# amansanghvi/Thesis

Measured on AMD Instinct MI355X. Metric: particle-updates/sec (particles x scans/s) @1081 beams, higher is better.
Workload: dtype int8 map cells (lattice log-odds), f64 poses/weights; 1 GPU; BASELINE configs[2]: room16 synthetic, 4096 particles/GPU, 1081 beams, 0.05 m grid, K=30 samples, both matcher stages, resample every step; particles_per_gpu=4096, beams=1081, parallelism=particles sharded x1

## Files before the change

### include/rbpf_hip.h

```cpp
#ifndef RBPF_HIP_H
#define RBPF_HIP_H

#include <stdint.h>

#ifdef __cplusplus
extern "C" {
#endif

#define RBPF_OK 0
#define RBPF_EINVAL (-1)
#define RBPF_ENOMEM (-2)
#define RBPF_EDEVICE (-3)
#define RBPF_ESTATE (-4)
#define RBPF_ERANGE (-5)

#define RBPF_IMU_UNICYCLE 0
#define RBPF_IMU_ABSOLUTE 1
#define RBPF_IMU_VELOCITY 2

typedef struct rbpf_handle rbpf_handle;

typedef struct rbpf_config {
    int32_t n_particles;
    int32_t n_samples;
// ... 110 lines not shown
int32_t rbpf_pack_raw_width(rbpf_handle* h);
int32_t rbpf_pack_meta_width(rbpf_handle* h);
int  rbpf_gather_pack_meta(rbpf_handle* h, const int32_t* local_idx, int32_t n, void* d_raw);
int  rbpf_meta_from_raw(rbpf_handle* h, const int32_t* raw, int32_t n, int32_t* meta_out, int64_t* bytes_out);
int  rbpf_pack_particles_raw(rbpf_handle* h, const int32_t* local_idx, int32_t n, const int32_t* raw, void* d_buf,
                             int64_t cap_bytes, int64_t* bytes_out);

int  rbpf_get_poses(rbpf_handle* h, double* out_p3);
int  rbpf_get_covs(rbpf_handle* h, double* out_p9);
int  rbpf_get_weights(rbpf_handle* h, double* out_p);
int  rbpf_set_state(rbpf_handle* h, const double* poses_p3, const double* covs_p9,
                    const double* weights_p);
int  rbpf_get_rng_state(rbpf_handle* h, uint64_t* scan_updates, uint64_t* resample_draws);
int  rbpf_set_rng_state(rbpf_handle* h, uint64_t scan_updates, uint64_t resample_draws);
int  rbpf_get_tile_count(rbpf_handle* h, int32_t particle, int32_t* out_n);
int  rbpf_get_tile(rbpf_handle* h, int32_t particle, int32_t k, double* centre2, int8_t* cells);
int  rbpf_set_tile(rbpf_handle* h, int32_t particle, double cx, double cy, const int8_t* cells);
int  rbpf_get_dim(rbpf_handle* h, int32_t* out_dim);
int  rbpf_get_odds_at(rbpf_handle* h, int32_t particle, const double* xy, int32_t n,
                      double* out_vals, uint8_t* out_none);

#define RBPF_RENDER_DEVICE_OUT 1u
int  rbpf_map_extent(rbpf_handle* h, int32_t particle, int32_t* box4);
int  rbpf_render_map(rbpf_handle* h, int32_t particle, const int32_t* box4, const double* weights,
                     uint32_t flags, int8_t* cells, float* prob, float* occ_frac);

#define RBPF_LOAD_DEVICE_IN 1u
int  rbpf_load_map(rbpf_handle* h, int32_t particle, const int32_t* box4, const int8_t* cells, uint32_t flags);
#define RBPF_PLACE_DEVICE_IN  1u
#define RBPF_PLACE_DEVICE_OUT 2u
// ... 102 lines not shown
```

### thesis_amd/_lib.py

```python
from __future__ import annotations

import ctypes as C
import os

HERE = os.path.dirname(os.path.abspath(__file__))
LIB_PATH = os.path.join(HERE, "librbpf_hip.so")

RBPF_OK = 0
RBPF_EINVAL, RBPF_ENOMEM, RBPF_EDEVICE, RBPF_ESTATE, RBPF_ERANGE = -1, -2, -3, -4, -5
RBPF_RENDER_DEVICE_OUT = 1
RBPF_LOAD_DEVICE_IN = 1
RBPF_CAST_DEVICE_OUT = 1
RBPF_LOCATE_DEVICE_OUT = 1
RBPF_ALIGN_DEVICE_OUT = 1
RBPF_GAIN_DEVICE_OUT = 1
RBPF_TRAVEL_DEVICE_OUT, RBPF_TRAVEL_THROUGH_UNKNOWN = 1, 2
RBPF_FRONTIER_DEVICE_OUT = 1
RBPF_SCORE_DEVICE_IN, RBPF_SCORE_DEVICE_OUT, RBPF_SCORE_FIELDS = 1, 2, 13
RBPF_W_UNIFORM, RBPF_W_RESAMPLE, RBPF_W_GIVEN = 0, 1, 2
RBPF_EST_F64, RBPF_EST_I32 = 16, 4
RBPF_TRACK_IMU, RBPF_TRACK_SCAN, RBPF_TRACK_CHUNK, RBPF_TRACK_DEVICE_OUT = 1, 2, 64, 1
RBPF_BUILD_DEVICE_OUT, RBPF_BUILD_ACCUMULATE = 1, 2
RBPF_REFINE_DEVICE_OUT = 1
RBPF_PAIRS_DEVICE_OUT = 1
# ... 76 lines not shown
    "rbpf_apply_resample_local": (C.c_int, [_H, _I, _I]),
    "rbpf_set_global_ids": (C.c_int, [_H, _I]),
    "rbpf_pack_meta_width": (C.c_int32, [_H]),
    "rbpf_unpack_particles": (C.c_int, [_H, _I, C.c_int32, C.c_void_p, _I]),
    "rbpf_pack_raw_width": (C.c_int32, [_H]),
    "rbpf_gather_pack_meta": (C.c_int, [_H, _I, C.c_int32, C.c_void_p]),
    "rbpf_meta_from_raw": (C.c_int, [_H, _I, C.c_int32, _I, C.POINTER(C.c_int64)]),
    "rbpf_pack_particles_raw": (C.c_int, [_H, _I, C.c_int32, _I, C.c_void_p, C.c_int64, C.POINTER(C.c_int64)]),
    "rbpf_get_poses": (C.c_int, [_H, _D]),
    "rbpf_get_covs": (C.c_int, [_H, _D]),
    "rbpf_get_weights": (C.c_int, [_H, _D]),
    "rbpf_set_state": (C.c_int, [_H, _D, _D, _D]),
    "rbpf_get_rng_state": (C.c_int, [_H, C.POINTER(C.c_uint64), C.POINTER(C.c_uint64)]),
    "rbpf_set_rng_state": (C.c_int, [_H, C.c_uint64, C.c_uint64]),
    "rbpf_get_tile_count": (C.c_int, [_H, C.c_int32, _I]),
    "rbpf_get_tile": (C.c_int, [_H, C.c_int32, C.c_int32, _D, _B]),
    "rbpf_set_tile": (C.c_int, [_H, C.c_int32, C.c_double, C.c_double, _B]),
    "rbpf_get_dim": (C.c_int, [_H, _I]),
    "rbpf_get_odds_at": (C.c_int, [_H, C.c_int32, _D, C.c_int32, _D, _U]),
    "rbpf_map_extent": (C.c_int, [_H, C.c_int32, _I]),
    "rbpf_render_map": (C.c_int, [_H, C.c_int32, _I, _D, C.c_uint32, C.c_void_p, C.c_void_p, C.c_void_p]),
    "rbpf_load_map": (C.c_int, [_H, C.c_int32, _I, C.c_void_p, C.c_uint32]),
    "rbpf_place_map": (C.c_int, [_H, C.c_int32, _I, C.c_void_p, C.c_int32, C.c_int32, C.c_double, _D, C.c_int32, C.c_int32, C.c_uint32,
                       C.c_void_p, C.c_void_p]),
    "rbpf_set_map_updates": (C.c_int, [_H, C.c_int32]),
    "rbpf_get_map_updates": (C.c_int, [_H, _I]),
    "rbpf_get_map_update_workgroups": (C.c_int, [_H, _I]),
    "rbpf_cast_scans": (C.c_int, [_H, C.c_int32, _D, C.c_int32, _D, C.c_int32, C.c_double, C.c_uint32, C.c_void_p, C.c_void_p]),
    "rbpf_locate_scan": (C.c_int, [_H, C.c_int32, _I, _D, _D, C.c_int32, C.c_int32, C.c_uint32, C.c_void_p, C.c_void_p]),
    "rbpf_align_points": (C.c_int, [_H, C.c_int32, _I, _D, C.c_int32, _D, C.c_int32, C.c_int32, C.c_int32, C.c_int32, C.c_uint32,
# ... 86 lines not shown
```

### thesis_amd/csrc/kernels_resample.hip

```cpp
#include <limits.h>

#include "rbpf_internal.h"

namespace rbpf {

static const int PLAN_THREADS = 1024;

__device__ __forceinline__ dd dd_two_prod(double a, double b) {
    double p = a * b;
    double e = __fma_rn(a, b, -p);
    return {p, e};
}
__device__ __forceinline__ dd dd_mul_d(dd a, double b) {
    dd p = dd_two_prod(a.hi, b);
    double lo = p.lo + a.lo * b;
    double hi = p.hi + lo;
    return {hi, lo - (hi - p.hi)};
}
__device__ __forceinline__ dd dd_sub(dd a, dd b) { return dd_add(a, dd{-b.hi, -b.lo}); }
__device__ __forceinline__ dd dd_div_d(dd a, double b) {
    double q1 = a.hi / b;
    dd r = dd_sub(a, dd_two_prod(q1, b));
    double q2 = (r.hi + r.lo) / b;
    double hi = q1 + q2;
// ... 447 lines not shown
    if (tid == 0) { v.tile_bbox[4 * td + 0] = j.x0; v.tile_bbox[4 * td + 1] = j.x1; v.tile_bbox[4 * td + 2] = j.ya; v.tile_bbox[4 * td + 3] = j.yb - 1; }
}

__global__ __launch_bounds__(PLAN_THREADS) void resample_plan_kernel(ResampleArgs a) { resample_plan_stage(a); }
__global__ void resample_expand_kernel(int P, const int32_t* __restrict__ T, int32_t* __restrict__ idx) {
    const int j = blockIdx.x * blockDim.x + threadIdx.x;
    if (j < P) resample_expand_one(P, T, idx, j);
}
__global__ __launch_bounds__(PLAN_THREADS) void resample_pair_kernel(PairArgs a) { resample_pair_stage(a); }
__global__ __launch_bounds__(PLAN_THREADS) void sources_to_T_kernel(int P, const int32_t* __restrict__ idx, int32_t* __restrict__ T,
                                                                     int32_t* __restrict__ did) { sources_to_T_stage(P, idx, T, did); }

enum { RS_PLAN = 1, RS_SRC2T = 2, RS_EXPAND = 4, RS_PAIR = 8, RS_GATHER = 16 };
static const int RS_FUSE_MAX = 4096;
static const int RS_GATHER_FUSE_MAX = 1024;
struct FusedArgs { int stages; ResampleArgs ra; int32_t* idx; PairArgs pa; GatherArgs ga; };
__global__ __launch_bounds__(PLAN_THREADS) void resample_fused_kernel(FusedArgs f) {
    extern __shared__ __align__(16) int32_t s_dyn[];
    int32_t* const s_T = s_dyn; int32_t* const s_idx = s_dyn + RS_FUSE_MAX;
    const int tid = threadIdx.x, P = f.ra.P;
#ifdef RBPF_STAMPS
    long long st[6]; st[0] = clock64();
#define RSTAMP(k) st[k] = clock64()
#else
#define RSTAMP(k) do { } while (0)
#endif
    if (f.stages & RS_PLAN) { resample_plan_stage(f.ra); __syncthreads(); }
    RSTAMP(1);
    if (f.stages & RS_SRC2T) { sources_to_T_stage(P, f.idx, f.ra.T, f.ra.did); __syncthreads(); }
    for (int j = tid; j < P; j += PLAN_THREADS) s_T[j] = f.ra.T[j];
    __syncthreads();
    if (f.stages & RS_EXPAND) { for (int j = tid; j < P; j += PLAN_THREADS) { resample_expand_one(P, s_T, s_idx, j); f.idx[j] = s_idx[j]; } }
    else for (int j = tid; j < P; j += PLAN_THREADS) s_idx[j] = f.idx[j];
    __syncthreads();
    RSTAMP(2);
    if (f.stages & RS_PAIR) { PairArgs pa = f.pa; pa.T = s_T; pa.idx = s_idx; resample_pair_stage(pa); __syncthreads(); }
    RSTAMP(3);
    if (f.stages & RS_GATHER) { GatherArgs ga = f.ga; ga.T = s_T; ga.idx = s_idx; for (int j = tid; j < ga.P; j += PLAN_THREADS) resample_gather_one(ga, j); }
    RSTAMP(4);
#ifdef RBPF_STAMPS
    if (tid == 0) printf("resample_fused: plan %lld expand %lld pair %lld gather %lld cycles\n", st[1] - st[0], st[2] - st[1], st[3] - st[2], st[4] - st[3]);
#endif
}

static void launch_resample_fused(const FusedArgs& f, hipStream_t s) {
    const size_t lds = 2 * RS_FUSE_MAX * sizeof(int32_t);
    static size_t lds_set[MAX_DEVICES] = {};
    ensure_dynamic_lds(reinterpret_cast<const void*>(resample_fused_kernel), lds, lds_set);
    hipLaunchKernelGGL(resample_fused_kernel, dim3(1), dim3(PLAN_THREADS), lds, s, f);
}

void launch_export_weights(const DevView& v, double* d_out, int n_global, const uint8_t* d_bad, hipStream_t s) {
    (void)hipMemsetAsync(d_out, 0, (size_t)(n_global + (d_bad ? 1 : 0)) * 8, s);
    hipLaunchKernelGGL(export_weights_kernel, dim3((v.P + 255) / 256), dim3(256), 0, s, v.P, v.weight, v.global_id, d_out, n_global, d_bad);
// ... 3 lines not shown
    hipLaunchKernelGGL(gather_meta_kernel, dim3((tot + 255) / 256), dim3(256), 0, s, v, d_local, n, d_out);
}
void launch_pack(const DevView& v, const void* d_jobs, int n_jobs, void* d_buf, hipStream_t s) {
    if (n_jobs) hipLaunchKernelGGL(pack_kernel, dim3(n_jobs), dim3(BLOCK), 0, s, v, static_cast<const PackJob*>(d_jobs), static_cast<unsigned char*>(d_buf));
}
void launch_unpack(const DevView& v, const ResampleBuffers& b, const void* d_jobs, int n_jobs, const void* d_buf, hipStream_t s) {
    if (n_jobs) hipLaunchKernelGGL(unpack_kernel, dim3(n_jobs), dim3(BLOCK), 0, s, v, static_cast<const UnpackJob*>(d_jobs),
                                   static_cast<const unsigned char*>(d_buf), b.pending_free, b.n_pending);
    hipLaunchKernelGGL(resample_release_kernel, dim3(1), dim3(256), 0, s, v, b.pending_free, b.n_pending);
}

void launch_resample_indices(int P, const double* d_w, double u, double spread, int32_t* d_T, int32_t* d_idx,
                             int32_t* d_did, int32_t* d_err, hipStream_t s) {
    ResampleArgs ra{P, d_w, u, spread, d_T, d_did, d_err};
    if (P <= RS_FUSE_MAX) {
        FusedArgs f{RS_PLAN | RS_EXPAND, ra, d_idx, PairArgs{}, GatherArgs{}};
        launch_resample_fused(f, s);
        return;
    }
    hipLaunchKernelGGL(resample_plan_kernel, dim3(1), dim3(PLAN_THREADS), 0, s, ra);
    hipLaunchKernelGGL(resample_expand_kernel, dim3((P + 255) / 256), dim3(256), 0, s, P, d_T, d_idx);
}

void launch_resample_local(const DevView& v, const ResampleBuffers& b, const double* d_w, double u, double spread, hipStream_t s) {
    const PairArgs pa{v.P, b.T, b.idx, b.did, v.slot, b.slot2, b.dead_list, b.jobs, b.n_jobs, v.err};
    const GatherArgs ga{v.P, b.idx, b.did, v.px, v.py, v.pth, v.cov, v.weight, b.px2, b.py2, b.pth2, b.cov2, b.w2, b.T, v.dup_of};
    const bool fuse_gather = v.P <= RS_GATHER_FUSE_MAX;
    if (v.P > RS_FUSE_MAX) {
        if (d_w) launch_resample_indices(v.P, d_w, u, spread, b.T, b.idx, b.did, v.err, s);
        else hipLaunchKernelGGL(sources_to_T_kernel, dim3(1), dim3(PLAN_THREADS), 0, s, v.P, b.idx, b.T, b.did);
        hipLaunchKernelGGL(resample_pair_kernel, dim3(1), dim3(PLAN_THREADS), 0, s, pa);
    } else {
        FusedArgs f{(d_w ? RS_PLAN | RS_EXPAND : RS_SRC2T) | RS_PAIR | (fuse_gather ? RS_GATHER : 0),
                    ResampleArgs{v.P, d_w, u, spread, b.T, b.did, v.err}, b.idx, pa, ga};
        launch_resample_fused(f, s);
    }
    CopyArgs ca{v, b.jobs, b.n_jobs, b.pending_free, b.n_pending, fuse_gather ? 0 : 1, ga};
    hipLaunchKernelGGL(resample_copy_kernel, dim3(512), dim3(COPY_BLOCK), 0, s, ca);
    hipLaunchKernelGGL(resample_release_kernel, dim3(1), dim3(256), 0, s, v, b.pending_free, b.n_pending);
}

}
```

### thesis_amd/csrc/rbpf_api.hip

```cpp
#include <math.h>
#include <stdio.h>
#include <stdlib.h>
#include <string.h>

#include <algorithm>
#include <limits>

#include "rbpf_host.h"

using namespace rbpf;

static thread_local std::string g_create_err;

#define HIP_TRY(h, call)                                                                           \
    do {                                                                                           \
        hipError_t e_ = (call);                                                                    \
        if (e_ != hipSuccess) {                                                                    \
            (h)->err = std::string(#call) + ": " + hipGetErrorString(e_);                          \
            return RBPF_EDEVICE;                                                                   \
        }                                                                                          \
    } while (0)

struct DevGuard {
    int prev = -1; bool switched = false;
    explicit DevGuard(int dev) {
        if (hipGetDevice(&prev) != hipSuccess) { (void)hipGetLastError(); prev = -1; }
        if (prev != dev) { if (hipSetDevice(dev) == hipSuccess) switched = prev >= 0; else (void)hipGetLastError(); }
    }
    ~DevGuard() { if (switched) (void)hipSetDevice(prev); }
    DevGuard(const DevGuard&) = delete; DevGuard& operator=(const DevGuard&) = delete;
};
#define ON_DEVICE(h) DevGuard dev_guard_((h)->cfg.device)

static int fail(rbpf_handle* h, int code, const std::string& msg) {
    if (h) h->err = msg; else g_create_err = msg;
    return code;
}

template <typename T>
static int dev_alloc(rbpf_handle* h, T** out, size_t n) {
    h->allocs.emplace_back();
    hipError_t e = h->allocs.back().reserve(n * sizeof(T));
    if (e != hipSuccess) { h->err = std::string("hipMalloc: ") + hipGetErrorString(e); return RBPF_ENOMEM; }
    *out = h->allocs.back().as<T>();
    return RBPF_OK;
}
#define ALLOC(h, ptr, n) do { int rc_ = dev_alloc(h, &(ptr), (n)); if (rc_) return rc_; } while (0)
// ... 125 lines not shown
            double rel = pos - (double)lat * v.tile_len;
            int cidx = trunc_to_int(rel / v.cs + (double)dim / 2.0);
            if (cidx < 0 || cidx >= dim) { delete h; return fail(nullptr, RBPF_EINVAL, "cell index formula leaves the tile for this cell_size (the reference would raise IndexError)"); }
            if (g_first == INT32_MAX) g_first = g;
            uint32_t ent = ((uint32_t)(lat + v.R) << 16) | (uint32_t)cidx;
            if (!lut.empty() && ent < lut.back()) { delete h; return fail(nullptr, RBPF_EINVAL, "cell index formula is not monotone for this cell_size"); }
            lut.push_back(ent);
        }
        v.g_min = g_first; v.n_lut = (int)lut.size();
    }

    int rc = RBPF_OK;
    auto build = [&]() -> int {
        HIP_TRY(h, hipStreamCreateWithFlags(&h->stream, hipStreamNonBlocking));
        h->own_stream = true;
        for (int k = 0; k < rbpf_handle::N_KERN; ++k)
            for (int e = 0; e < 2; ++e) {
                h->ring[k][e].resize(rbpf_handle::RING);
                for (auto& ev : h->ring[k][e]) HIP_TRY(h, h->events.create(&ev, hipEventDisableSystemFence));
                h->begin_used[k].assign(rbpf_handle::RING, nullptr);
            }
        const size_t P = v.P, LL = (size_t)v.L * v.L, cells = (size_t)dim * dim;
        uint32_t* d_lut; ALLOC(h, d_lut, h->h_lut.size()); v.lut = d_lut;
        HIP_TRY(h, hipMemcpy(d_lut, h->h_lut.data(), h->h_lut.size() * 4, hipMemcpyHostToDevice));
        {
            const int KW = (dim + WIN - 1) / WIN;
            std::vector<int32_t> gw((size_t)v.L * (KW + 1));
            for (int a = 0; a < v.L; ++a)
                for (int k = 0; k <= KW; ++k) {
                    uint32_t key = k < KW ? (((uint32_t)a << 16) | (uint32_t)(k * WIN)) : ((uint32_t)(a + 1) << 16);
// ... 22 lines not shown
            v.wsel_x = reinterpret_cast<const float*>(d + 3 * MBP * 8 + 4 * MBP * 4 + MBP); v.wsel_y = v.wsel_x + MBW;
            v.wsel_idx = reinterpret_cast<const uint16_t*>(v.wsel_y + MBW);
            HIP_TRY(h, h->rings[R_SCAN].create(h->scan_bytes));
            HIP_TRY(h, h->rings[R_LAST].create(MB * 16));
            HIP_TRY(h, h->rings[R_IDX].create((size_t)P * 8));
        }
        ALLOC(h, v.upd_pose, 3 * P);
        ALLOC(h, v.prop_prep, 24 * P);
        ALLOC(h, v.prop_samp, 256 * P);
        ALLOC(h, v.stats, ST_COUNT); ALLOC(h, v.err, 1);
        ALLOC(h, v.mu_fallback, P); HIP_TRY(h, hipMemset(v.mu_fallback, 0, P * 4));
        ALLOC(h, v.ev_queue, 2); HIP_TRY(h, hipMemset(v.ev_queue, 0, 8));
        ALLOC(h, h->d_did_early, 1);
        HIP_TRY(h, hipMemset(h->d_did_early, 0, 4));
        HIP_TRY(h, h->events.create(&h->ev_weights, hipEventDisableTiming | hipEventDisableSystemFence));
        {
            v.mu_mode = env_is("RBPF_MAP_KERNEL", "window") ? MU_WINDOW : env_is("RBPF_MAP_KERNEL", "ray") ? MU_RAY : env_is("RBPF_MAP_KERNEL", "ev") ? MU_EV : MU_DEFAULT;
            v.ev_resident = env_is("RBPF_EV_RESIDENT", "0") ? 0 : 1;
            const char* eg = getenv("RBPF_EV_GRID");
            v.ev_grid = eg ? std::max(0, atoi(eg)) : 0;
            v.match_stage_slow = env_is("RBPF_MATCH_STAGE", "slow") ? 1 : 0;
            const char* ws = getenv("RBPF_WSAFE");
            v.wsafe_override = ws ? (float)atof(ws) : -1.0f;
            v.weight_entry_f64 = env_is("RBPF_WEIGHT_ENTRY", "f64") ? 1 : 0;
            v.ndt_refine = h->cfg.ndt_refine;
            h->dedup_enabled = !env_is("RBPF_MATCH_DEDUP", "0");
        }
        ALLOC(h, v.dup_of, P); v.dups_valid = 0;
        ALLOC(h, h->d_last_xy, 2 * (size_t)c.max_beams); ALLOC(h, h->d_tmp_sel, 2 * (size_t)c.max_beams);
        if (raycast_lds_bytes(c.max_beams, v.reach) > LDS_LIMIT) return fail(h, RBPF_EINVAL, "max_beams too large for the LDS window layout");
        match_geometry(c, c.cell_size, h->mN, h->mds, h->mmcs, h->md0, h->mncr);
        h->mlds = match_lds_bytes(h->mN, c.max_beams, match_max_coarse(h->mncr, 0.7, h->mmcs), match_per_rot(0.7, h->mmcs));
        if (h->mlds > LDS_LIMIT) return fail(h, RBPF_EINVAL, "matcher region does not fit in LDS for this cell_size");
        if (c.ndt_refine && ndt_cells(h->mmcs) >= 2) {
            if (ndt_lds_bytes(h->mN, c.max_beams) > LDS_LIMIT) return fail(h, RBPF_EINVAL, "NDT stage: matcher region does not fit in LDS");
            ALLOC(h, v.ndt_occ, P * (size_t)h->mN * (h->mN / 32)); ALLOC(h, v.ndt_aux, 5 * P);
        }
        ALLOC(h, h->d_match, 13 * P); ALLOC(h, h->d_bad, P); ALLOC(h, h->d_guess_full, P * (size_t)c.n_samples * 3);
        {
            ResampleBuffers& r = h->rs;
            ALLOC(h, r.T, P); ALLOC(h, r.idx, P); ALLOC(h, r.did, 1); ALLOC(h, r.slot2, P); ALLOC(h, r.dead_list, P);
            ALLOC(h, r.jobs, 2 * P); ALLOC(h, r.n_jobs, 2); ALLOC(h, r.pending_free, (size_t)v.pool_tiles); ALLOC(h, r.n_pending, 1);
            ALLOC(h, r.px2, P); ALLOC(h, r.py2, P); ALLOC(h, r.pth2, P); ALLOC(h, r.cov2, 9 * P); ALLOC(h, r.w2, P);
            HIP_TRY(h, hipMemset(r.n_pending, 0, 4)); HIP_TRY(h, hipMemset(r.n_jobs, 0, 8)); HIP_TRY(h, hipMemset(r.did, 0, 4));
        }
        HIP_TRY(h, hipMemset(v.pool, 0, (size_t)v.pool_tiles * cells));
        HIP_TRY(h, hipMemset(v.px, 0, P * 8)); HIP_TRY(h, hipMemset(v.py, 0, P * 8)); HIP_TRY(h, hipMemset(v.pth, 0, P * 8));
        HIP_TRY(h, hipMemset(v.cov, 0, 9 * P * 8));
        HIP_TRY(h, hipMemset(v.stats, 0, ST_COUNT * 8)); HIP_TRY(h, hipMemset(v.err, 0, 4));
        std::vector<double> w(P, 1.0);
        HIP_TRY(h, hipMemcpy(v.weight, w.data(), P * 8, hipMemcpyHostToDevice));
        std::vector<int32_t> ids(P), tab(P * LL, -1), fs(v.pool_tiles), bb((size_t)v.pool_tiles * 4);
        for (size_t p = 0; p < P; ++p) { ids[p] = (int32_t)p; tab[p * LL + (size_t)v.R * v.L + v.R] = (int32_t)p; }
        for (int t = 0; t < v.pool_tiles; ++t) { bb[4 * t] = INT32_MAX; bb[4 * t + 1] = -1; bb[4 * t + 2] = INT32_MAX; bb[4 * t + 3] = -1; }
        int32_t top = v.pool_tiles - (int32_t)P;
        for (int i = 0; i < top; ++i) fs[i] = v.pool_tiles - 1 - i;
        HIP_TRY(h, hipMemcpy(v.slot, ids.data(), P * 4, hipMemcpyHostToDevice));
        HIP_TRY(h, hipMemcpy(v.global_id, ids.data(), P * 4, hipMemcpyHostToDevice));
        HIP_TRY(h, hipMemcpy(v.tile_tab, tab.data(), P * LL * 4, hipMemcpyHostToDevice));
        HIP_TRY(h, hipMemcpy(v.free_stack, fs.data(), (size_t)v.pool_tiles * 4, hipMemcpyHostToDevice));
        HIP_TRY(h, hipMemcpy(v.free_top, &top, 4, hipMemcpyHostToDevice));
        HIP_TRY(h, hipMemcpy(v.tile_bbox, bb.data(), bb.size() * 4, hipMemcpyHostToDevice));
        return RBPF_OK;
    };
    rc = build();
    if (rc != RBPF_OK) { g_create_err = h->err; rbpf_destroy(h); return rc; }
    *out = h;
    return RBPF_OK;
}

int rbpf_destroy(rbpf_handle* h) {
    if (!h) return RBPF_OK;
    ON_DEVICE(h);
    if (hipStreamSynchronize(h->stream) != hipSuccess) (void)hipGetLastError();
    h->each_staging([](Staging& s) { if (s.wait() != hipSuccess) (void)hipGetLastError(); });
    if (h->ev_weights_valid && hipEventSynchronize(h->ev_weights) != hipSuccess) (void)hipGetLastError();
    for (Block& b : h->allocs) b.release();
    for (Block& b : h->buf) b.release();
    for (Block& b : h->track_mem) b.release();
    h->each_staging([](Staging& s) { s.release(); });
    h->each_staging([](Staging& s) { s.destroy_event(); });
    h->events.destroy();
    if (h->own_stream && h->stream) (void)hipStreamDestroy(h->stream);
    (void)hipGetLastError();
    delete h;
    return RBPF_OK;
}

const char* rbpf_last_error(const rbpf_handle* h) { return h ? h->err.c_str() : g_create_err.c_str(); }

int rbpf_set_stream(rbpf_handle* h, void* s) {
    if (!h) return RBPF_EINVAL;
    ON_DEVICE(h);
    HIP_TRY(h, hipStreamSynchronize(h->stream));
    if (h->own_stream && h->stream) (void)hipStreamDestroy(h->stream);
    h->own_stream = false;
    h->stream = static_cast<hipStream_t>(s);
    h->last_end = nullptr;
    return RBPF_OK;
}

int rbpf_release_stream(rbpf_handle* h) {
    if (!h) return RBPF_EINVAL;
    ON_DEVICE(h);
    if (h->own_stream) return RBPF_OK;
    HIP_TRY(h, hipStreamSynchronize(h->stream));
    if (h->early_n > 0) HIP_TRY(h, h->stage[S_EARLY].wait());
    h->stream = nullptr;
    HIP_TRY(h, hipStreamCreateWithFlags(&h->stream, hipStreamNonBlocking));
    h->own_stream = true;
    h->last_end = nullptr;
    return RBPF_OK;
}

int rbpf_abi_struct_bytes(int32_t* config_bytes, int32_t* counters_bytes) {
    if (config_bytes) *config_bytes = (int32_t)sizeof(rbpf_config);
    if (counters_bytes) *counters_bytes = (int32_t)sizeof(rbpf_counters);
    return RBPF_OK;
}

int rbpf_synchronize(rbpf_handle* h) {
    if (!h) return RBPF_EINVAL;
// ... 247 lines not shown
    }
    const double* d_g = nullptr;
    if (guesses) {
        HIP_TRY(h, hipMemcpyAsync(h->d_guess_full, guesses, P * (size_t)v.K * 3 * 8, hipMemcpyHostToDevice, h->stream));
        d_g = h->d_guess_full;
    }
    if (!match_override && !guesses) h->prof_begin_chained(1); else h->prof_begin(1);
    const int32_t* match_of = (!match_override && v.dups_valid) ? v.dup_of : nullptr;
    if (h->prop_capture && !h->d_prop_w) ALLOC(h, h->d_prop_w, P * (size_t)v.K);
    launch_propose_weight(v, h->d_match, match_of, d_g, h->d_bad, h->cfg.seed, (uint32_t)h->scan_updates, h->prop_capture ? h->d_prop_w : nullptr, h->stream);
    h->prop_valid = true; h->prop_captured = h->prop_capture;
    v.dups_valid = 0;
    h->prof_end(1);
    HIP_TRY(h, hipGetLastError());
    h->ev_weights_valid = false;
    if (h->record_ev_weights) { HIP_TRY(h, hipEventRecord(h->ev_weights, h->stream)); h->ev_weights_valid = true; }
    h->scan_begun = true; h->begin_seen = true;
    return RBPF_OK;
}

int rbpf_scan_update_end(rbpf_handle* h) {
    if (!h) return RBPF_EINVAL;
    ON_DEVICE(h);
    if (!h->scan_begun) return fail(h, RBPF_ESTATE, "rbpf_scan_update_begin has not been called");
    h->scan_begun = false;
    if (!h->map_updates) {
        launch_bad_weight(h->v, h->d_bad, h->stream);
        HIP_TRY(h, hipGetLastError());
        h->scan_updates++;
    } else {
        const int rc = run_map_update(h, h->d_bad);
        if (rc) return rc;
    }
    if (h->track_on && (h->track_flags & RBPF_TRACK_SCAN)) return track_record(h, true);
    return RBPF_OK;
}

int rbpf_set_proposal_capture(rbpf_handle* h, int32_t on) {
    if (!h) return RBPF_EINVAL;
    h->prop_capture = on != 0;
// ... 148 lines not shown

static double internal_uniform(rbpf_handle* h) {
    uint64_t z = h->cfg.seed + 0x9E3779B97F4A7C15ull * (++h->resample_draws);
    z = (z ^ (z >> 30)) * 0xBF58476D1CE4E5B9ull;
    z = (z ^ (z >> 27)) * 0x94D049BB133111EBull;
    z ^= z >> 31;
    return (double)(z >> 11) * (1.0 / 9007199254740992.0);
}

static void swap_state_buffers(rbpf_handle* h) {
    DevView& v = h->v; ResampleBuffers& r = h->rs;
    std::swap(v.px, r.px2); std::swap(v.py, r.py2); std::swap(v.pth, r.pth2);
    std::swap(v.cov, r.cov2); std::swap(v.weight, r.w2); std::swap(v.slot, r.slot2);
}

static int resample_local(rbpf_handle* h, const double* d_w, double u, double spread) {
    DevView& v = h->v;
    h->prof_begin(2);
    launch_resample_local(v, h->rs, d_w, u, spread, h->stream);
    h->prof_end(2);
    HIP_TRY(h, hipGetLastError());
    swap_state_buffers(h);
    if (h->track_on) {
        launch_track_compose(v.P, h->rs.did, h->rs.idx, h->track_pending(h->track_cur), h->track_pending(h->track_cur ^ 1), h->stream);
        HIP_TRY(h, hipGetLastError());
        h->track_cur ^= 1;
    }
    v.dups_valid = h->dedup_enabled ? 1 : 0;
    if (h->match_rows == 2) h->match_rows = 0;
    return RBPF_OK;
}

int rbpf_resample(rbpf_handle* h, double u, int32_t* idx_out, int32_t* did_resample) {
    if (!h) return RBPF_EINVAL;
    ON_DEVICE(h);
    DevView& v = h->v;
    if (u != u) u = internal_uniform(h);
    if (!(u >= 0.0 && u < 1.0)) return fail(h, RBPF_EINVAL, "u must lie in [0, 1)");
    int rc = resample_local(h, v.weight, u, h->cfg.resample_spread);
    if (rc) return rc;
    if (idx_out) HIP_TRY(h, hipMemcpyAsync(idx_out, h->rs.idx, (size_t)v.P * 4, hipMemcpyDeviceToHost, h->stream));
    if (did_resample) HIP_TRY(h, hipMemcpyAsync(did_resample, h->rs.did, 4, hipMemcpyDeviceToHost, h->stream));
    if (idx_out || did_resample) return check_device_error(h);
    return RBPF_OK;
}

int rbpf_set_global_ids(rbpf_handle* h, const int32_t* ids) {
    if (!h || !ids) return RBPF_EINVAL;
    ON_DEVICE(h);
    HIP_TRY(h, hipMemcpyAsync(h->v.global_id, ids, (size_t)h->v.P * 4, hipMemcpyHostToDevice, h->stream));
    HIP_TRY(h, hipStreamSynchronize(h->stream));
    return RBPF_OK;
}

// ... 318 lines not shown
int rbpf_set_rng_state(rbpf_handle* h, uint64_t scan_updates, uint64_t resample_draws) {
    if (!h) return RBPF_EINVAL;
    h->scan_updates = scan_updates; h->resample_draws = resample_draws;
    return RBPF_OK;
}

int rbpf_get_tile_count(rbpf_handle* h, int32_t particle, int32_t* out_n) {
    if (!h || !out_n) return RBPF_EINVAL;
    ON_DEVICE(h);
    std::vector<int32_t> tab;
    int rc = fetch_tab(h, particle, tab);
    if (rc) return rc;
    int n = 0;
    for (int32_t t : tab) n += t >= 0;
    *out_n = n;
    return RBPF_OK;
}

int rbpf_get_tile(rbpf_handle* h, int32_t particle, int32_t k, double* centre2, int8_t* cells) {
    if (!h || !centre2 || !cells) return RBPF_EINVAL;
    ON_DEVICE(h);
    std::vector<int32_t> tab;
    int rc = fetch_tab(h, particle, tab);
    if (rc) return rc;
    const DevView& v = h->v;
    int n = 0;
    for (int a = 0; a < v.L; ++a)
        for (int b = 0; b < v.L; ++b) {
            int32_t t = tab[(size_t)a * v.L + b];
            if (t < 0) continue;
// ... 1576 lines not shown
```

### thesis_amd/csrc/rbpf_host.h

```cpp
#pragma once
#include <stdlib.h>
#include <algorithm>
#include <string>
#include <vector>

#include "rbpf_internal.h"

static const size_t LDS_LIMIT = 160 * 1024;

enum MemKind { MEM_DEVICE, MEM_PINNED, MEM_PAGEABLE };
struct Block {
    MemKind kind = MEM_DEVICE;
    unsigned char* p = nullptr; size_t cap = 0;
    hipError_t reserve(size_t bytes) {
        if (p && cap >= bytes) return hipSuccess;
        release();
        const size_t want = kind == MEM_PINNED ? std::max<size_t>(bytes * 2, 1 << 16) : std::max<size_t>(bytes, 4096);
        hipError_t e = hipSuccess;
        if (kind == MEM_DEVICE) e = hipMalloc(reinterpret_cast<void**>(&p), want);
        else if (kind == MEM_PINNED) e = hipHostMalloc(reinterpret_cast<void**>(&p), want, hipHostMallocDefault);
        else if (!(p = static_cast<unsigned char*>(malloc(want)))) e = hipErrorOutOfMemory;
        if (e == hipSuccess) cap = want; else p = nullptr;
        return e;
    }
// ... 76 lines not shown
                              {{MEM_PAGEABLE}, hipEventDisableTiming}, {{MEM_PAGEABLE}, hipEventDisableTiming}, {{MEM_PAGEABLE}, hipEventDisableTiming},
                              {{MEM_PAGEABLE}, hipEventDisableTiming}, {{MEM_PAGEABLE}, hipEventDisableTiming}, {{MEM_PAGEABLE}, hipEventDisableTiming},
                              {{MEM_PAGEABLE}, hipEventDisableTiming}, {{MEM_PINNED}, hipEventDisableTiming}, {{MEM_PINNED}, hipEventDisableTiming},
                              {{MEM_PAGEABLE}, hipEventDisableTiming}, {{MEM_PAGEABLE}, hipEventDisableTiming}, {{MEM_PAGEABLE}, hipEventDisableTiming},
                              {{MEM_PAGEABLE}, hipEventDisableTiming}, {{MEM_PAGEABLE}, hipEventDisableTiming}, {{MEM_PAGEABLE}, hipEventDisableTiming}};
    hipError_t reserve(int b, size_t bytes) {
        if (buf[b].cap >= bytes) return hipSuccess;
        if (b >= B_DRAIN_FIRST) { const hipError_t e = hipStreamSynchronize(stream); if (e != hipSuccess) return e; }
        return buf[b].reserve(bytes);
    }
    PinnedRing rings[R_COUNT];
    EventPool events;
    template <typename F> void each_staging(F f) { for (Staging& s : stage) f(s); for (PinnedRing& r : rings) for (Staging& s : r.slot) f(s); }
    hipEvent_t ev_weights = nullptr; bool ev_weights_valid = false, record_ev_weights = false, begin_seen = false;
    int32_t* d_did_early = nullptr; bool scan_begun = false;
    int early_n = 0;
    unsigned char* d_scan = nullptr; size_t scan_bytes = 0;
    template <typename T> T* in_slot(unsigned char* slot, const T* dev) const { return reinterpret_cast<T*>(slot + (reinterpret_cast<const unsigned char*>(dev) - d_scan)); }
    int mN = 0, mds = 1, mncr = 0; double mmcs = 0, md0 = 0; size_t mlds = 0;
    double* d_last_xy = nullptr; float* d_tmp_sel = nullptr;
    int n_last_dev = -1;
    int match_rows = 0;
    double* d_match = nullptr; uint8_t* d_bad = nullptr; double* d_guess_full = nullptr;
    unsigned long long resample_draws = 0;
    int ev_workgroups = 0;
    bool map_updates = true;
    static const int N_KERN = 5, RING = 512;
    std::vector<hipEvent_t> ring[N_KERN][2];
    int ring_n[N_KERN] = {0, 0, 0, 0, 0};
    std::vector<hipEvent_t> begin_used[N_KERN];
// ... 27 lines not shown
```

### thesis_amd/csrc/rbpf_internal.h

```cpp
#pragma once
#include <hip/hip_runtime.h>
#include <stdint.h>
#include <mutex>

#include "../../include/rbpf_hip.h"
#include "rbpf_math.h"
#include "rbpf_blockrelax.h"

namespace rbpf {

static const int MAX_DEVICES = 16;
inline void ensure_dynamic_lds(const void* fn, size_t bytes, size_t* set) {
    static std::mutex mu;
    std::lock_guard<std::mutex> lock(mu);
    int dev = 0;
    (void)hipGetDevice(&dev);
    const bool tracked = dev >= 0 && dev < MAX_DEVICES;
    if (tracked && bytes <= set[dev]) return;
    const hipError_t rc = hipFuncSetAttribute(fn, hipFuncAttributeMaxDynamicSharedMemorySize, (int)bytes);
    if (rc != hipSuccess) { (void)hipGetLastError(); return; }
    if (tracked) set[dev] = bytes;
}


// ... 48 lines not shown
    int ndt_refine;
    int32_t* dup_of; int dups_valid;
    float wsafe_override;
    int weight_entry_f64;
    int match_stage_slow;
    unsigned long long* stats;
    int32_t* err;
};

struct ResampleBuffers {
    int32_t *T, *idx, *did;
    int32_t *slot2, *dead_list, *jobs;
    int32_t *n_jobs;
    int32_t *pending_free, *n_pending;
    double *px2, *py2, *pth2, *cov2, *w2;
};

enum { ST_RAY_CELLS = 0, ST_CELLS_WRITTEN = 1, ST_GATHERS = 2, ST_SLOW_CELLS = 3,
       ST_COPIES = 4, ST_COPY_BYTES = 5, ST_WINDOW_FALLBACKS = 6, ST_FALLBACK_REASONS = 7,
       ST_NDT_RUNS = 16, ST_NDT_EVALS = 17, ST_NDT_ACCEPTED = 18, ST_MATCH_SHARED = 19, ST_MAP_WINDOWS = 20,
       ST_FB_BOUND = 21, ST_FB_TABLES = 22, ST_MAP_EVENTS = 23, ST_EV_OVERFLOWS = 24, ST_COUNT = 28 };

struct RenderJob {
    int32_t pos;
    int32_t i0, j0;
    int32_t ni, jlo, jhi;
    int32_t ox, oy;
};
struct RenderFilter {
    const RenderJob* jobs;
    const double* lut;
// ... 208 lines not shown
void launch_ingest(const void* mapped_src, void* d_dst, size_t bytes, hipStream_t s);
void launch_ingest2(const int32_t* mapped_a, int32_t* d_a, const int32_t* mapped_b, int32_t* d_b, int n, hipStream_t s);
void launch_readback(void* mapped_dst, const double* d_nan_elem, const int32_t* d_did, const int32_t* d_idx, int n, hipStream_t s);
bool map_update_ray_available(const DevView& v);
void launch_map_update_ray(const DevView& v, const int32_t* only, hipStream_t s, hipEvent_t t0 = nullptr, hipEvent_t t1 = nullptr);
bool map_update_ev_available(const DevView& v);
int launch_map_update_ev(const DevView& v, hipStream_t s, hipEvent_t t0 = nullptr, hipEvent_t t1 = nullptr);
void launch_get_odds(const DevView& v, int particle, const double* d_xy, int n, double* d_vals,
                     uint8_t* d_none, hipStream_t s);
void launch_last_scan(const DevView& v, int particle, double* d_out_xy, hipStream_t s);
void launch_imu_update(const DevView& v, int model, double d0, double d1, double d2, double dt_ticks,
                       const double* vel_noise, hipStream_t s);
void launch_resample_indices(int P, const double* d_w, double u, double spread, int32_t* d_T, int32_t* d_idx,
                             int32_t* d_did, int32_t* d_err, hipStream_t s);
void launch_resample_local(const DevView& v, const ResampleBuffers& b, const double* d_w, double u, double spread, hipStream_t s);
void launch_export_weights(const DevView& v, double* d_out, int n_global, const uint8_t* d_bad, hipStream_t s);
void launch_gather_meta(const DevView& v, const int32_t* d_local, int n, int32_t* d_out, hipStream_t s);
void launch_pack(const DevView& v, const void* d_jobs, int n_jobs, void* d_buf, hipStream_t s);
void launch_unpack(const DevView& v, const ResampleBuffers& b, const void* d_jobs, int n_jobs, const void* d_buf, hipStream_t s);
struct PackJobHost { int32_t particle, tile, x0, x1, ya, yb; long long off; };
struct UnpackJobHost { int32_t particle, pos, has, x0, x1, ya, yb, pad; long long off; };
void launch_propose_weight(const DevView& v, const double* d_match, const int32_t* d_match_of, const double* d_guesses, uint8_t* d_bad,
                           uint64_t seed, uint32_t stream, double* d_dbg_w, hipStream_t s);
void launch_bad_weight(const DevView& v, const uint8_t* d_bad, hipStream_t s);
size_t match_lds_bytes(int N, int B, int n_coarse, int per_rot);
int match_sc_capacity(int N, int B, size_t lds);
int match_per_rot(double max_range_m, double mcs);
size_t ndt_lds_bytes(int N, int B);
int ndt_cells(double mcs);
void match_geometry(const rbpf_config& c, double cell_size, int& N, int& ds, double& mcs, double& d0, int& n_coarse_rot);
// ... 45 lines not shown
```

### thesis_amd/engine.py

```python
from __future__ import annotations

import atexit
import ctypes as C
import sys
import weakref
from typing import Any, Dict, List, NamedTuple, Optional, Tuple

import numpy as np

from . import _lib
from ._lib import RbpfConfig, RbpfCounters, IMU_UNICYCLE, IMU_ABSOLUTE, IMU_VELOCITY

IMU_MODEL_IDS = {"unicycle": IMU_UNICYCLE, "absolute": IMU_ABSOLUTE, "velocity": IMU_VELOCITY}


def _dp(a: np.ndarray):
    return a.ctypes.data_as(C.POINTER(C.c_double))


def _ip(a: np.ndarray):
    return a.ctypes.data_as(C.POINTER(C.c_int32))


def _f64(a) -> np.ndarray:
# ... 343 lines not shown
        c = None if covs is None else _f64(np.broadcast_to(covs, (self.P, 3, 3)))
        w = None if weights is None else _f64(np.broadcast_to(weights, (self.P,)))
        self._check(self._lib.rbpf_set_state(self._h, None if p is None else _dp(p),
                                             None if c is None else _dp(c), None if w is None else _dp(w)))

    def tiles(self, particle: int) -> List[Tuple[Tuple[float, float], np.ndarray]]:
        n = C.c_int32()
        self._check(self._lib.rbpf_get_tile_count(self._h, particle, C.byref(n)))
        out = []
        for k in range(n.value):
            c = np.empty(2)
            cells = np.empty((self.dim, self.dim), dtype=np.int8)
            self._check(self._lib.rbpf_get_tile(self._h, particle, k, _dp(c), cells.ctypes.data_as(C.POINTER(C.c_int8))))
            out.append(((float(c[0]), float(c[1])), cells))
        return out

    def set_tile(self, particle: int, centre, cells: np.ndarray):
        cells = np.ascontiguousarray(cells, dtype=np.int8)
        if cells.shape != (self.dim, self.dim):
            raise ValueError("tile must be [dim, dim] int8")
        self._check(self._lib.rbpf_set_tile(self._h, particle, float(centre[0]), float(centre[1]),
                                            cells.ctypes.data_as(C.POINTER(C.c_int8))))

    def load_map(self, raster, particle: Optional[int] = None):
        cfg = self.cfg
        for name, have, want in (("cell_size", raster.cell_size, cfg.cell_size), ("quantum", raster.quantum, cfg.quantum),
                                 ("tile_len", raster.tile_len, float(cfg.tile_len_m)), ("dim", raster.dim, self.dim)):
            if abs(float(have) - float(want)) > 1e-9 * abs(float(want)):
                raise ValueError(f"raster {name} = {have!r} differs from the engine's {want!r}")
        if raster.cells is None:
# ... 950 lines not shown
```

Baseline: 2.256 million particle-updates/s.

## Plan resampling early on a side stream overlapping the scan update tail

```diff
diff --git a/include/rbpf_hip.h b/include/rbpf_hip.h
--- a/include/rbpf_hip.h
+++ b/include/rbpf_hip.h
@@ -148,6 +148,7 @@
 int  rbpf_get_rng_state(rbpf_handle* h, uint64_t* scan_updates, uint64_t* resample_draws);
 int  rbpf_set_rng_state(rbpf_handle* h, uint64_t scan_updates, uint64_t resample_draws);
 int  rbpf_get_tile_count(rbpf_handle* h, int32_t particle, int32_t* out_n);
+int  rbpf_get_pool_state(rbpf_handle* h, int32_t* free_top, int32_t* free_stack, int32_t* words3, int32_t* tile_ids);
 int  rbpf_get_tile(rbpf_handle* h, int32_t particle, int32_t k, double* centre2, int8_t* cells);
 int  rbpf_set_tile(rbpf_handle* h, int32_t particle, double cx, double cy, const int8_t* cells);
 int  rbpf_get_dim(rbpf_handle* h, int32_t* out_dim);
diff --git a/thesis_amd/_lib.py b/thesis_amd/_lib.py
--- a/thesis_amd/_lib.py
+++ b/thesis_amd/_lib.py
@@ -114,6 +114,7 @@
     "rbpf_get_rng_state": (C.c_int, [_H, C.POINTER(C.c_uint64), C.POINTER(C.c_uint64)]),
     "rbpf_set_rng_state": (C.c_int, [_H, C.c_uint64, C.c_uint64]),
     "rbpf_get_tile_count": (C.c_int, [_H, C.c_int32, _I]),
+    "rbpf_get_pool_state": (C.c_int, [_H, _I, _I, _I, _I]),
     "rbpf_get_tile": (C.c_int, [_H, C.c_int32, C.c_int32, _D, _B]),
     "rbpf_set_tile": (C.c_int, [_H, C.c_int32, C.c_double, C.c_double, _B]),
     "rbpf_get_dim": (C.c_int, [_H, _I]),
diff --git a/thesis_amd/csrc/kernels_resample.hip b/thesis_amd/csrc/kernels_resample.hip
--- a/thesis_amd/csrc/kernels_resample.hip
+++ b/thesis_amd/csrc/kernels_resample.hip
@@ -485,7 +485,10 @@
 enum { RS_PLAN = 1, RS_SRC2T = 2, RS_EXPAND = 4, RS_PAIR = 8, RS_GATHER = 16 };
 static const int RS_FUSE_MAX = 4096;
 static const int RS_GATHER_FUSE_MAX = 1024;
-struct FusedArgs { int stages; ResampleArgs ra; int32_t* idx; PairArgs pa; GatherArgs ga; };
+struct FusedArgs {
+    int stages; ResampleArgs ra; int32_t* idx; PairArgs pa; GatherArgs ga;
+    int mode; const uint8_t* bad; int32_t* early;
+};
 __global__ __launch_bounds__(PLAN_THREADS) void resample_fused_kernel(FusedArgs f) {
     extern __shared__ __align__(16) int32_t s_dyn[];
     int32_t* const s_T = s_dyn; int32_t* const s_idx = s_dyn + RS_FUSE_MAX;
@@ -496,6 +499,13 @@
 #else
 #define RSTAMP(k) do { } while (0)
 #endif
+    if (f.mode == RS_MODE_EARLY) {
+        int any = 0;
+        for (int j = tid; j < P; j += PLAN_THREADS) any |= f.bad[j];
+        if (__syncthreads_or(any)) { if (tid == 0) *f.early = 0; return; }
+    } else if (f.mode == RS_MODE_UNLESS_EARLY) {
+        if (*f.early) return;
+    }
     if (f.stages & RS_PLAN) { resample_plan_stage(f.ra); __syncthreads(); }
     RSTAMP(1);
     if (f.stages & RS_SRC2T) { sources_to_T_stage(P, f.idx, f.ra.T, f.ra.did); __syncthreads(); }
@@ -509,6 +519,7 @@
     RSTAMP(3);
     if (f.stages & RS_GATHER) { GatherArgs ga = f.ga; ga.T = s_T; ga.idx = s_idx; for (int j = tid; j < ga.P; j += PLAN_THREADS) resample_gather_one(ga, j); }
     RSTAMP(4);
+    if (f.mode == RS_MODE_EARLY && tid == 0) *f.early = 1;
 #ifdef RBPF_STAMPS
     if (tid == 0) printf("resample_fused: plan %lld expand %lld pair %lld gather %lld cycles\n", st[1] - st[0], st[2] - st[1], st[3] - st[2], st[4] - st[3]);
 #endif
@@ -542,7 +553,7 @@
                              int32_t* d_did, int32_t* d_err, hipStream_t s) {
     ResampleArgs ra{P, d_w, u, spread, d_T, d_did, d_err};
     if (P <= RS_FUSE_MAX) {
-        FusedArgs f{RS_PLAN | RS_EXPAND, ra, d_idx, PairArgs{}, GatherArgs{}};
+        FusedArgs f{RS_PLAN | RS_EXPAND, ra, d_idx, PairArgs{}, GatherArgs{}, RS_MODE_INLINE, nullptr, nullptr};
         launch_resample_fused(f, s);
         return;
     }
@@ -550,22 +561,37 @@
     hipLaunchKernelGGL(resample_expand_kernel, dim3((P + 255) / 256), dim3(256), 0, s, P, d_T, d_idx);
 }
 
-void launch_resample_local(const DevView& v, const ResampleBuffers& b, const double* d_w, double u, double spread, hipStream_t s) {
+static GatherArgs gather_args(const DevView& v, const ResampleBuffers& b) {
+    return GatherArgs{v.P, b.idx, b.did, v.px, v.py, v.pth, v.cov, v.weight, b.px2, b.py2, b.pth2, b.cov2, b.w2, b.T, v.dup_of};
+}
+static bool gather_fused(const DevView& v) { return v.P <= RS_GATHER_FUSE_MAX; }
+
+static const int RS_EARLY_MIN = 2048;
+bool resample_plan_early_available(const DevView& v, bool any_size) { return v.P <= RS_FUSE_MAX && (any_size || v.P >= RS_EARLY_MIN); }
+
+void launch_resample_plan(const DevView& v, const ResampleBuffers& b, const double* d_w, double u, double spread, int mode,
+                          const uint8_t* d_bad, hipStream_t s) {
     const PairArgs pa{v.P, b.T, b.idx, b.did, v.slot, b.slot2, b.dead_list, b.jobs, b.n_jobs, v.err};
-    const GatherArgs ga{v.P, b.idx, b.did, v.px, v.py, v.pth, v.cov, v.weight, b.px2, b.py2, b.pth2, b.cov2, b.w2, b.T, v.dup_of};
-    const bool fuse_gather = v.P <= RS_GATHER_FUSE_MAX;
     if (v.P > RS_FUSE_MAX) {
         if (d_w) launch_resample_indices(v.P, d_w, u, spread, b.T, b.idx, b.did, v.err, s);
         else hipLaunchKernelGGL(sources_to_T_kernel, dim3(1), dim3(PLAN_THREADS), 0, s, v.P, b.idx, b.T, b.did);
         hipLaunchKernelGGL(resample_pair_kernel, dim3(1), dim3(PLAN_THREADS), 0, s, pa);
     } else {
-        FusedArgs f{(d_w ? RS_PLAN | RS_EXPAND : RS_SRC2T) | RS_PAIR | (fuse_gather ? RS_GATHER : 0),
-                    ResampleArgs{v.P, d_w, u, spread, b.T, b.did, v.err}, b.idx, pa, ga};
+        FusedArgs f{(d_w ? RS_PLAN | RS_EXPAND : RS_SRC2T) | RS_PAIR | (gather_fused(v) ? RS_GATHER : 0),
+                    ResampleArgs{v.P, d_w, u, spread, b.T, b.did, v.err}, b.idx, pa, gather_args(v, b), mode, d_bad, b.early};
         launch_resample_fused(f, s);
     }
-    CopyArgs ca{v, b.jobs, b.n_jobs, b.pending_free, b.n_pending, fuse_gather ? 0 : 1, ga};
+}
+
+void launch_resample_apply(const DevView& v, const ResampleBuffers& b, hipStream_t s) {
+    CopyArgs ca{v, b.jobs, b.n_jobs, b.pending_free, b.n_pending, gather_fused(v) ? 0 : 1, gather_args(v, b)};
     hipLaunchKernelGGL(resample_copy_kernel, dim3(512), dim3(COPY_BLOCK), 0, s, ca);
     hipLaunchKernelGGL(resample_release_kernel, dim3(1), dim3(256), 0, s, v, b.pending_free, b.n_pending);
 }
 
-}
+void launch_resample_local(const DevView& v, const ResampleBuffers& b, const double* d_w, double u, double spread, hipStream_t s) {
+    launch_resample_plan(v, b, d_w, u, spread, RS_MODE_INLINE, nullptr, s);
+    launch_resample_apply(v, b, s);
+}
+
+}
diff --git a/thesis_amd/csrc/rbpf_api.hip b/thesis_amd/csrc/rbpf_api.hip
--- a/thesis_amd/csrc/rbpf_api.hip
+++ b/thesis_amd/csrc/rbpf_api.hip
@@ -30,7 +30,7 @@
     ~DevGuard() { if (switched) (void)hipSetDevice(prev); }
     DevGuard(const DevGuard&) = delete; DevGuard& operator=(const DevGuard&) = delete;
 };
-#define ON_DEVICE(h) DevGuard dev_guard_((h)->cfg.device)
+#define ON_DEVICE(h) DevGuard dev_guard_((h)->cfg.device); ++(h)->api_calls
 
 static int fail(rbpf_handle* h, int code, const std::string& msg) {
     if (h) h->err = msg; else g_create_err = msg;
@@ -186,6 +186,7 @@
     auto build = [&]() -> int {
         HIP_TRY(h, hipStreamCreateWithFlags(&h->stream, hipStreamNonBlocking));
         h->own_stream = true;
+        HIP_TRY(h, hipStreamCreateWithFlags(&h->side_stream, hipStreamNonBlocking));
         for (int k = 0; k < rbpf_handle::N_KERN; ++k)
             for (int e = 0; e < 2; ++e) {
                 h->ring[k][e].resize(rbpf_handle::RING);
@@ -238,6 +239,7 @@
         ALLOC(h, h->d_did_early, 1);
         HIP_TRY(h, hipMemset(h->d_did_early, 0, 4));
         HIP_TRY(h, h->events.create(&h->ev_weights, hipEventDisableTiming | hipEventDisableSystemFence));
+        HIP_TRY(h, h->events.create(&h->ev_planned, hipEventDisableTiming | hipEventDisableSystemFence));
         {
             v.mu_mode = env_is("RBPF_MAP_KERNEL", "window") ? MU_WINDOW : env_is("RBPF_MAP_KERNEL", "ray") ? MU_RAY : env_is("RBPF_MAP_KERNEL", "ev") ? MU_EV : MU_DEFAULT;
             v.ev_resident = env_is("RBPF_EV_RESIDENT", "0") ? 0 : 1;
@@ -249,6 +251,7 @@
             v.weight_entry_f64 = env_is("RBPF_WEIGHT_ENTRY", "f64") ? 1 : 0;
             v.ndt_refine = h->cfg.ndt_refine;
             h->dedup_enabled = !env_is("RBPF_MATCH_DEDUP", "0");
+            h->plan_early = env_is("RBPF_RS_EARLY", "0") ? 0 : env_is("RBPF_RS_EARLY", "always") ? 2 : 1;
         }
         ALLOC(h, v.dup_of, P); v.dups_valid = 0;
         ALLOC(h, h->d_last_xy, 2 * (size_t)c.max_beams); ALLOC(h, h->d_tmp_sel, 2 * (size_t)c.max_beams);
@@ -266,7 +269,9 @@
             ALLOC(h, r.T, P); ALLOC(h, r.idx, P); ALLOC(h, r.did, 1); ALLOC(h, r.slot2, P); ALLOC(h, r.dead_list, P);
             ALLOC(h, r.jobs, 2 * P); ALLOC(h, r.n_jobs, 2); ALLOC(h, r.pending_free, (size_t)v.pool_tiles); ALLOC(h, r.n_pending, 1);
             ALLOC(h, r.px2, P); ALLOC(h, r.py2, P); ALLOC(h, r.pth2, P); ALLOC(h, r.cov2, 9 * P); ALLOC(h, r.w2, P);
+            ALLOC(h, r.early, 1);
             HIP_TRY(h, hipMemset(r.n_pending, 0, 4)); HIP_TRY(h, hipMemset(r.n_jobs, 0, 8)); HIP_TRY(h, hipMemset(r.did, 0, 4));
+            HIP_TRY(h, hipMemset(r.early, 0, 4));
         }
         HIP_TRY(h, hipMemset(v.pool, 0, (size_t)v.pool_tiles * cells));
         HIP_TRY(h, hipMemset(v.px, 0, P * 8)); HIP_TRY(h, hipMemset(v.py, 0, P * 8)); HIP_TRY(h, hipMemset(v.pth, 0, P * 8));
@@ -297,6 +302,7 @@
     if (!h) return RBPF_OK;
     ON_DEVICE(h);
     if (hipStreamSynchronize(h->stream) != hipSuccess) (void)hipGetLastError();
+    if (h->side_stream && hipStreamSynchronize(h->side_stream) != hipSuccess) (void)hipGetLastError();
     h->each_staging([](Staging& s) { if (s.wait() != hipSuccess) (void)hipGetLastError(); });
     if (h->ev_weights_valid && hipEventSynchronize(h->ev_weights) != hipSuccess) (void)hipGetLastError();
     for (Block& b : h->allocs) b.release();
@@ -306,6 +312,7 @@
     h->each_staging([](Staging& s) { s.destroy_event(); });
     h->events.destroy();
     if (h->own_stream && h->stream) (void)hipStreamDestroy(h->stream);
+    if (h->side_stream) (void)hipStreamDestroy(h->side_stream);
     (void)hipGetLastError();
     delete h;
     return RBPF_OK;
@@ -317,10 +324,12 @@
     if (!h) return RBPF_EINVAL;
     ON_DEVICE(h);
     HIP_TRY(h, hipStreamSynchronize(h->stream));
+    HIP_TRY(h, hipStreamSynchronize(h->side_stream));
     if (h->own_stream && h->stream) (void)hipStreamDestroy(h->stream);
     h->own_stream = false;
     h->stream = static_cast<hipStream_t>(s);
     h->last_end = nullptr;
+    h->ev_weights_valid = false;
     return RBPF_OK;
 }
 
@@ -330,6 +339,8 @@
     if (h->own_stream) return RBPF_OK;
     HIP_TRY(h, hipStreamSynchronize(h->stream));
     if (h->early_n > 0) HIP_TRY(h, h->stage[S_EARLY].wait());
+    HIP_TRY(h, hipStreamSynchronize(h->side_stream));
+    h->ev_weights_valid = false;
     h->stream = nullptr;
     HIP_TRY(h, hipStreamCreateWithFlags(&h->stream, hipStreamNonBlocking));
     h->own_stream = true;
@@ -607,8 +618,9 @@
     h->prof_end(1);
     HIP_TRY(h, hipGetLastError());
     h->ev_weights_valid = false;
-    if (h->record_ev_weights) { HIP_TRY(h, hipEventRecord(h->ev_weights, h->stream)); h->ev_weights_valid = true; }
+    if (h->record_ev_weights || (h->plan_early && resample_plan_early_available(v, h->plan_early == 2))) { HIP_TRY(h, hipEventRecord(h->ev_weights, h->stream)); h->ev_weights_valid = true; }
     h->scan_begun = true; h->begin_seen = true;
+    h->weighted_at = h->api_calls;
     return RBPF_OK;
 }
 
@@ -617,6 +629,7 @@
     ON_DEVICE(h);
     if (!h->scan_begun) return fail(h, RBPF_ESTATE, "rbpf_scan_update_begin has not been called");
     h->scan_begun = false;
+    h->weighted_at = h->weighted_at + 1 == h->api_calls ? h->api_calls : 0;
     if (!h->map_updates) {
         launch_bad_weight(h->v, h->d_bad, h->stream);
         HIP_TRY(h, hipGetLastError());
@@ -795,10 +808,19 @@
     std::swap(v.cov, r.cov2); std::swap(v.weight, r.w2); std::swap(v.slot, r.slot2);
 }
 
-static int resample_local(rbpf_handle* h, const double* d_w, double u, double spread) {
+static int resample_local(rbpf_handle* h, const double* d_w, double u, double spread, bool clean = false) {
     DevView& v = h->v;
+    const bool early = clean && d_w && h->plan_early && h->ev_weights_valid && !h->scan_begun && resample_plan_early_available(v, h->plan_early == 2);
+    if (early) {
+        HIP_TRY(h, hipStreamWaitEvent(h->side_stream, h->ev_weights, 0));
+        launch_resample_plan(v, h->rs, d_w, u, spread, RS_MODE_EARLY, h->d_bad, h->side_stream);
+        HIP_TRY(h, hipEventRecord(h->ev_planned, h->side_stream));
+        h->early_plans++;
+    }
     h->prof_begin(2);
-    launch_resample_local(v, h->rs, d_w, u, spread, h->stream);
+    if (early) HIP_TRY(h, hipStreamWaitEvent(h->stream, h->ev_planned, 0));
+    launch_resample_plan(v, h->rs, d_w, u, spread, early ? RS_MODE_UNLESS_EARLY : RS_MODE_INLINE, nullptr, h->stream);
+    launch_resample_apply(v, h->rs, h->stream);
     h->prof_end(2);
     HIP_TRY(h, hipGetLastError());
     swap_state_buffers(h);
@@ -818,7 +840,9 @@
     DevView& v = h->v;
     if (u != u) u = internal_uniform(h);
     if (!(u >= 0.0 && u < 1.0)) return fail(h, RBPF_EINVAL, "u must lie in [0, 1)");
-    int rc = resample_local(h, v.weight, u, h->cfg.resample_spread);
+    const bool clean = h->weighted_at != 0 && h->weighted_at + 1 == h->api_calls;
+    h->weighted_at = 0;
+    int rc = resample_local(h, v.weight, u, h->cfg.resample_spread, clean);
     if (rc) return rc;
     if (idx_out) HIP_TRY(h, hipMemcpyAsync(idx_out, h->rs.idx, (size_t)v.P * 4, hipMemcpyDeviceToHost, h->stream));
     if (did_resample) HIP_TRY(h, hipMemcpyAsync(did_resample, h->rs.did, 4, hipMemcpyDeviceToHost, h->stream));
@@ -1167,6 +1191,29 @@
     int n = 0;
     for (int32_t t : tab) n += t >= 0;
     *out_n = n;
+    return RBPF_OK;
+}
+
+int rbpf_get_pool_state(rbpf_handle* h, int32_t* free_top, int32_t* free_stack, int32_t* words3, int32_t* tile_ids) {
+    if (!h) return RBPF_EINVAL;
+    ON_DEVICE(h);
+    const DevView& v = h->v;
+    const size_t LL = (size_t)v.L * v.L;
+    std::vector<int32_t> slot((size_t)v.P), tab(tile_ids ? (size_t)v.P * LL : 0);
+    if (free_top) HIP_TRY(h, hipMemcpyAsync(free_top, v.free_top, 4, hipMemcpyDeviceToHost, h->stream));
+    if (free_stack) HIP_TRY(h, hipMemcpyAsync(free_stack, v.free_stack, (size_t)v.pool_tiles * 4, hipMemcpyDeviceToHost, h->stream));
+    if (words3) {
+        HIP_TRY(h, hipMemcpyAsync(words3, h->rs.n_pending, 4, hipMemcpyDeviceToHost, h->stream));
+        HIP_TRY(h, hipMemcpyAsync(words3 + 1, h->rs.early, 4, hipMemcpyDeviceToHost, h->stream));
+        words3[2] = (int32_t)h->early_plans;
+    }
+    if (tile_ids) {
+        HIP_TRY(h, hipMemcpyAsync(slot.data(), v.slot, slot.size() * 4, hipMemcpyDeviceToHost, h->stream));
+        HIP_TRY(h, hipMemcpyAsync(tab.data(), v.tile_tab, tab.size() * 4, hipMemcpyDeviceToHost, h->stream));
+    }
+    HIP_TRY(h, hipStreamSynchronize(h->stream));
+    if (tile_ids)
+        for (size_t p = 0; p < (size_t)v.P; ++p) memcpy(tile_ids + p * LL, tab.data() + (size_t)slot[p] * LL, LL * 4);
     return RBPF_OK;
 }
 
diff --git a/thesis_amd/csrc/rbpf_host.h b/thesis_amd/csrc/rbpf_host.h
--- a/thesis_amd/csrc/rbpf_host.h
+++ b/thesis_amd/csrc/rbpf_host.h
@@ -114,6 +114,10 @@
     template <typename F> void each_staging(F f) { for (Staging& s : stage) f(s); for (PinnedRing& r : rings) for (Staging& s : r.slot) f(s); }
     hipEvent_t ev_weights = nullptr; bool ev_weights_valid = false, record_ev_weights = false, begin_seen = false;
     int32_t* d_did_early = nullptr; bool scan_begun = false;
+    hipStream_t side_stream = nullptr; hipEvent_t ev_planned = nullptr; int plan_early = 1;
+    unsigned long long early_plans = 0;
+    unsigned long long api_calls = 0;
+    unsigned long long weighted_at = 0;
     int early_n = 0;
     unsigned char* d_scan = nullptr; size_t scan_bytes = 0;
     template <typename T> T* in_slot(unsigned char* slot, const T* dev) const { return reinterpret_cast<T*>(slot + (reinterpret_cast<const unsigned char*>(dev) - d_scan)); }
diff --git a/thesis_amd/csrc/rbpf_internal.h b/thesis_amd/csrc/rbpf_internal.h
--- a/thesis_amd/csrc/rbpf_internal.h
+++ b/thesis_amd/csrc/rbpf_internal.h
@@ -86,7 +86,9 @@
     int32_t *n_jobs;
     int32_t *pending_free, *n_pending;
     double *px2, *py2, *pth2, *cov2, *w2;
-};
+    int32_t *early;
+};
+enum { RS_MODE_INLINE = 0, RS_MODE_EARLY = 1, RS_MODE_UNLESS_EARLY = 2 };
 
 enum { ST_RAY_CELLS = 0, ST_CELLS_WRITTEN = 1, ST_GATHERS = 2, ST_SLOW_CELLS = 3,
        ST_COPIES = 4, ST_COPY_BYTES = 5, ST_WINDOW_FALLBACKS = 6, ST_FALLBACK_REASONS = 7,
@@ -325,6 +327,10 @@
 void launch_resample_indices(int P, const double* d_w, double u, double spread, int32_t* d_T, int32_t* d_idx,
                              int32_t* d_did, int32_t* d_err, hipStream_t s);
 void launch_resample_local(const DevView& v, const ResampleBuffers& b, const double* d_w, double u, double spread, hipStream_t s);
+bool resample_plan_early_available(const DevView& v, bool any_size);
+void launch_resample_plan(const DevView& v, const ResampleBuffers& b, const double* d_w, double u, double spread, int mode,
+                          const uint8_t* d_bad, hipStream_t s);
+void launch_resample_apply(const DevView& v, const ResampleBuffers& b, hipStream_t s);
 void launch_export_weights(const DevView& v, double* d_out, int n_global, const uint8_t* d_bad, hipStream_t s);
 void launch_gather_meta(const DevView& v, const int32_t* d_local, int n, int32_t* d_out, hipStream_t s);
 void launch_pack(const DevView& v, const void* d_jobs, int n_jobs, void* d_buf, hipStream_t s);
diff --git a/thesis_amd/engine.py b/thesis_amd/engine.py
--- a/thesis_amd/engine.py
+++ b/thesis_amd/engine.py
@@ -381,6 +381,13 @@
             self._check(self._lib.rbpf_get_tile(self._h, particle, k, _dp(c), cells.ctypes.data_as(C.POINTER(C.c_int8))))
             out.append(((float(c[0]), float(c[1])), cells))
         return out
+
+    def pool_state(self):
+        top, pend = C.c_int32(), np.zeros(3, dtype=np.int32)
+        stack = np.empty(int(self.cfg.pool_tiles), dtype=np.int32)
+        ids = np.empty((self.P, (2 * int(self.cfg.lattice_radius) + 1) ** 2), dtype=np.int32)
+        self._check(self._lib.rbpf_get_pool_state(self._h, C.byref(top), _ip(stack), _ip(pend), _ip(ids)))
+        return stack[:top.value].copy(), pend, ids
 
     def set_tile(self, particle: int, centre, cells: np.ndarray):
         cells = np.ascontiguousarray(cells, dtype=np.int8)
```

After: 2.271 million particle-updates/s (median of 6 runs). About the same (+0.7%).
